# 4ment/physher

Hardware: AMD Instinct MI355X
Metric: lnL+gradient evals/sec, 1000-taxon GTR+G4 fp64, 1e6 site patterns (higher is better)
Workload: dtype f64

## Files before the change

include/physher_amd.h:

```cpp
#ifndef PHYSHER_AMD_H
#define PHYSHER_AMD_H

#include <stddef.h>
#include <stdint.h>

#ifdef __cplusplus
extern "C" {
#endif

typedef struct phyamd_engine phyamd_engine;

enum {
	PHYAMD_OK = 0,
	PHYAMD_EINVAL = -1,
	PHYAMD_EDEVICE = -2,
	PHYAMD_ENOMEM = -3,
	PHYAMD_EUNSUPPORTED = -4
};

enum { PHYAMD_RESCALE_NEVER = 0, PHYAMD_RESCALE_ALWAYS = 1, PHYAMD_RESCALE_AUTO = 2 };

enum {
	PHYAMD_GRAD_FOLD_ROOT_FREQS = 1,
	PHYAMD_GRAD_COMPAT_SCALED = 2
// ... 44 lines not shown
int phyamd_gradient(phyamd_engine *e, int flags, double *lnl, double *cat_gradient);
int phyamd_branch_gradient(phyamd_engine *e, int flags, const double *rates_without_mu , double *lnl,
                           double *branch_gradient);
int phyamd_log_likelihood_device(phyamd_engine *e, double *device_out);
int phyamd_gradient_device(phyamd_engine *e, int flags, double *device_out);
int phyamd_root_invariant_term(phyamd_engine *e, double *out);

#define PHYAMD_MAX_PARAMETERS 2048
int phyamd_set_rate_matrix_derivatives(phyamd_engine *e, int count, const double *dQ);
int phyamd_parameter_gradient(phyamd_engine *e, int flags, double *lnl, double *cat_gradient, double *parameter_gradient);
int phyamd_parameter_gradient_device(phyamd_engine *e, int flags, double *device_out);
int phyamd_root_frequency_term(phyamd_engine *e, double *out );
int phyamd_branch_log_likelihood(phyamd_engine *e, int node, double length, double *lnl, double *d1, double *d2);
int phyamd_branch_hessian_diagonal(phyamd_engine *e, int flags, double *lnl, double *d1, double *d2);
int phyamd_branch_hessian_diagonal_device(phyamd_engine *e, int flags, double *device_out);
int phyamd_gradient_batch(phyamd_engine *e, int flags, int32_t count, const double *branch_lengths, double *lnl, double *cat_gradient);
int phyamd_gradient_batch_trees(phyamd_engine *e, int flags, int32_t count, const int32_t *left, const int32_t *right,
                                const int32_t *roots, const double *branch_lengths, double *lnl, double *cat_gradient);
typedef struct { int32_t items_fast, items_sequential, chunks; int64_t scratch_bytes; double ms; } phyamd_batch_profile;
int phyamd_get_batch_profile(phyamd_engine *e, phyamd_batch_profile *out);
int phyamd_nni_log_likelihoods(phyamd_engine *e, int flags, const double *central_lengths ,
                               double *lnl , double *d1 , double *d2 );
typedef struct { int32_t candidates; int64_t scratch_bytes; double ms; } phyamd_nni_profile;
int phyamd_get_nni_profile(phyamd_engine *e, phyamd_nni_profile *out);
int phyamd_spr_log_likelihoods(phyamd_engine *e, int flags, int32_t count, const int32_t *prune ,
                               double *lnl );
typedef struct { int32_t prunes, chunks; int64_t candidates, scratch_bytes; double ms; } phyamd_spr_profile;
int phyamd_get_spr_profile(phyamd_engine *e, phyamd_spr_profile *out);
int phyamd_synchronize(phyamd_engine *e);

int phyamd_get_pattern_log_likelihoods(phyamd_engine *e, double *out );
int phyamd_get_partials(phyamd_engine *e, int node, int upper, double *out);
int phyamd_get_node_matrices(phyamd_engine *e, int node, int derivative, double *out );
int phyamd_is_rescaling(phyamd_engine *e);
int phyamd_set_rescaling(phyamd_engine *e, int policy);
int phyamd_set_keep_partials(phyamd_engine *e, int on);

typedef struct {
	double matrices_ms, lower_ms, upper_ms, reduce_ms;
	int32_t lower_launches, upper_launches;
	int64_t device_bytes;
	int32_t tiles;
} phyamd_profile;
int phyamd_set_reduction_levels(phyamd_engine *e, int levels);
int phyamd_set_profiling(phyamd_engine *e, int on);
int phyamd_get_profile(phyamd_engine *e, phyamd_profile *out);

#ifdef __cplusplus
}
#endif
#endif
```

physher_amd/_lib.py:

```python
from __future__ import annotations

import ctypes as C
import os

_HERE = os.path.dirname(os.path.abspath(__file__))
LIB_PATH = os.environ.get("PHYAMD_LIB") or os.path.join(_HERE, "libphysher_amd.so")

ABI_VERSION = 5

OK, EINVAL, EDEVICE, ENOMEM, EUNSUPPORTED = 0, -1, -2, -3, -4
RESCALE_NEVER, RESCALE_ALWAYS, RESCALE_AUTO = 0, 1, 2
GRAD_FOLD_ROOT_FREQS, GRAD_COMPAT_SCALED = 1, 2


class Config(C.Structure):
    _fields_ = [
        ("tip_count", C.c_int32), ("pattern_count", C.c_int32), ("state_count", C.c_int32),
        ("category_count", C.c_int32), ("device", C.c_int32), ("rescale", C.c_int32),
        ("max_device_bytes", C.c_int64), ("stream", C.c_void_p),
    ]


class Profile(C.Structure):
    _fields_ = [
# ... 31 lines not shown
    ("phyamd_set_branch_lengths", C.c_int, [_P, _P]),
    ("phyamd_set_branch_length", C.c_int, [_P, C.c_int, C.c_double]),
    ("phyamd_update_all_nodes", C.c_int, [_P]),
    ("phyamd_set_eigen", C.c_int, [_P, _P, _P, _P]),
    ("phyamd_set_frequencies", C.c_int, [_P, _P]),
    ("phyamd_set_category_rates", C.c_int, [_P, _P, _P]),
    ("phyamd_set_node_matrices", C.c_int, [_P, C.c_int, _P]),
    ("phyamd_set_matrices", C.c_int, [_P, _P]),
    ("phyamd_set_rate_matrix", C.c_int, [_P, _P]),
    ("phyamd_log_likelihood", C.c_int, [_P, C.POINTER(C.c_double)]),
    ("phyamd_gradient", C.c_int, [_P, C.c_int, C.POINTER(C.c_double), _P]),
    ("phyamd_branch_gradient", C.c_int, [_P, C.c_int, _P, C.POINTER(C.c_double), _P]),
    ("phyamd_gradient_device", C.c_int, [_P, C.c_int, _P]),
    ("phyamd_log_likelihood_device", C.c_int, [_P, _P]),
    ("phyamd_root_invariant_term", C.c_int, [_P, C.POINTER(C.c_double)]),
    ("phyamd_set_rate_matrix_derivatives", C.c_int, [_P, C.c_int, _P]),
    ("phyamd_parameter_gradient", C.c_int, [_P, C.c_int, C.POINTER(C.c_double), _P, _P]),
    ("phyamd_parameter_gradient_device", C.c_int, [_P, C.c_int, _P]),
    ("phyamd_root_frequency_term", C.c_int, [_P, _P]),
    ("phyamd_branch_log_likelihood", C.c_int, [_P, C.c_int, C.c_double, C.POINTER(C.c_double), C.POINTER(C.c_double), C.POINTER(C.c_double)]),
    ("phyamd_branch_hessian_diagonal", C.c_int, [_P, C.c_int, C.POINTER(C.c_double), _P, _P]),
    ("phyamd_branch_hessian_diagonal_device", C.c_int, [_P, C.c_int, _P]),
    ("phyamd_gradient_batch", C.c_int, [_P, C.c_int, C.c_int32, _P, _P, _P]),
    ("phyamd_gradient_batch_trees", C.c_int, [_P, C.c_int, C.c_int32, _P, _P, _P, _P, _P, _P]),
    ("phyamd_get_batch_profile", C.c_int, [_P, C.POINTER(BatchProfile)]),
    ("phyamd_nni_log_likelihoods", C.c_int, [_P, C.c_int, _P, _P, _P, _P]),
    ("phyamd_get_nni_profile", C.c_int, [_P, C.POINTER(NniProfile)]),
    ("phyamd_spr_log_likelihoods", C.c_int, [_P, C.c_int, C.c_int32, _P, _P]),
    ("phyamd_get_spr_profile", C.c_int, [_P, C.POINTER(SprProfile)]),
    ("phyamd_synchronize", C.c_int, [_P]),
    ("phyamd_get_pattern_log_likelihoods", C.c_int, [_P, _P]),
    ("phyamd_get_partials", C.c_int, [_P, C.c_int, C.c_int, _P]),
    ("phyamd_get_node_matrices", C.c_int, [_P, C.c_int, C.c_int, _P]),
    ("phyamd_is_rescaling", C.c_int, [_P]),
    ("phyamd_set_rescaling", C.c_int, [_P, C.c_int]),
    ("phyamd_set_keep_partials", C.c_int, [_P, C.c_int]),
    ("phyamd_set_reduction_levels", C.c_int, [_P, C.c_int]),
    ("phyamd_set_profiling", C.c_int, [_P, C.c_int]),
    ("phyamd_get_profile", C.c_int, [_P, C.POINTER(Profile)]),
    ("phyamd_store", C.c_int, [_P]),
    ("phyamd_restore", C.c_int, [_P]),
    ("phyamd_compress_patterns", C.c_int, [C.c_int, C.c_int32, C.c_int64, _P, _P, C.POINTER(C.c_int32), _P, _P]),
]

_lib = None


def load():
    global _lib
    if _lib is not None:
        return _lib
    if not os.path.exists(LIB_PATH):
        raise ImportError(f"{LIB_PATH} is missing: build the HIP engine first (make -C physher_amd/csrc); there is no CPU fallback")
    lib = C.CDLL(LIB_PATH)
    for name, res, args in SYMBOLS:
        fn = getattr(lib, name)
        fn.restype = res
        fn.argtypes = args
    if lib.phyamd_abi_version() != ABI_VERSION:
        raise ImportError(f"ABI mismatch: library {lib.phyamd_abi_version()} != binding {ABI_VERSION}")
    _lib = lib
    return lib


class EngineError(RuntimeError):
    def __init__(self, code, message):
# ... 3 lines not shown
```

physher_amd/csrc/phyamd_abi.inc:

```

#include <condition_variable>
#include <functional>
#include <mutex>
#include <thread>

namespace {

class ShardWorkers {
public:
	explicit ShardWorkers(int n) : done_(0), generation_(0), stop_(false) {
		for (int i = 0; i < n; i++) threads_.emplace_back([this, i] { loop(i); });
	}
	~ShardWorkers() {
		{
			std::lock_guard<std::mutex> lk(m_);
			stop_ = true;
			generation_++;
		}
		cv_.notify_all();
		for (auto &t : threads_) t.join();
	}
	void run(const std::function<void(int)> &fn) {
		std::unique_lock<std::mutex> lk(m_);
		fn_ = &fn;
// ... 561 lines not shown
}


int phyamd_get_pattern_log_likelihoods(phyamd_engine *g, double *out) {
	CHECK_GROUP(g);
	if (!out) return fail(PHYAMD_EINVAL, "null out");
	return for_shards(g, [&](Shard *s, int i) { return shard_get_pattern_log_likelihoods(s, out + g->offset[i]); });
}

int phyamd_get_partials(phyamd_engine *g, int node, int upper, double *out) {
	CHECK_GROUP(g);
	if (group_size(g) == 1) return shard_get_partials(g->shards[0], node, upper, out);
	if (!out) return fail(PHYAMD_EINVAL, "null out");
	int rc;
	std::vector<std::vector<double>> part(group_size(g));
	if ((rc = for_shards(g, [&](Shard *s, int i) {
		     part[i].resize((size_t)g->C * s->P * g->S);
		     return shard_get_partials(s, node, upper, part[i].data());
	     })))
		return rc;
	for (int i = 0; i < group_size(g); i++) {
		const size_t ps = (size_t)(g->offset[i + 1] - g->offset[i]);
		for (int c = 0; c < g->C; c++)
			std::memcpy(out + ((size_t)c * g->P + g->offset[i]) * g->S, part[i].data() + (size_t)c * ps * g->S, sizeof(double) * ps * g->S);
	}
	return PHYAMD_OK;
}

int phyamd_get_node_matrices(phyamd_engine *g, int node, int derivative, double *out) {
	CHECK_GROUP(g);
	return shard_get_node_matrices(g->shards[0], node, derivative, out);
}

int phyamd_is_rescaling(phyamd_engine *g) {
	CHECK_GROUP(g);
	int any = 0;
	for (Shard *s : g->shards) any |= shard_is_rescaling(s);
	return any;
}

int phyamd_get_profile(phyamd_engine *g, phyamd_profile *out) {
	CHECK_GROUP(g);
	if (!out) return fail(PHYAMD_EINVAL, "null out");
	int rc;
	if ((rc = shard_get_profile(g->shards[0], out))) return rc;
	for (int i = 1; i < group_size(g); i++) {
		phyamd_profile p;
		if ((rc = shard_get_profile(g->shards[i], &p))) return rc;
		out->matrices_ms = std::max(out->matrices_ms, p.matrices_ms);
		out->lower_ms = std::max(out->lower_ms, p.lower_ms);
		out->upper_ms = std::max(out->upper_ms, p.upper_ms);
		out->reduce_ms = std::max(out->reduce_ms, p.reduce_ms);
		out->device_bytes += p.device_bytes;
		out->tiles = std::max(out->tiles, p.tiles);
	}
	return PHYAMD_OK;
}

}
```

physher_amd/csrc/phyamd_engine.hip:

```cpp

#include <hip/hip_runtime.h>
#include <hipcub/hipcub.hpp>

#include <algorithm>
#include <chrono>
#include <cmath>
#include <cstdarg>
#include <cstdio>
#include <cstdlib>
#include <cstring>
#include <string>
#include <vector>

#include "physher_amd.h"

#define PHYAMD_ABI_VERSION 5

namespace {

thread_local std::string g_last_error;

int fail(int code, const char *fmt, ...) {
	char buf[512];
	va_list ap;
	va_start(ap, fmt);
	vsnprintf(buf, sizeof buf, fmt, ap);
	va_end(ap);
	g_last_error = buf;
	return code;
}

#define HIP_TRY(expr)                                                                                       \
	do {                                                                                                    \
		hipError_t err__ = (expr);                                                                          \
		if (err__ != hipSuccess)                                                                            \
			return fail(err__ == hipErrorOutOfMemory ? PHYAMD_ENOMEM : PHYAMD_EDEVICE, "%s: %s (%s:%d)", #expr, \
			            hipGetErrorString(err__), __FILE__, __LINE__);                                      \
	} while (0)

constexpr int WAVE = 64;
constexpr int PPT_LOWER = 2, PPT_UPPER = 8;
constexpr int UPPER_MIN_WAVES = 6;
constexpr int MAX_WAVES = 16;
// ... 47 lines not shown
```

physher_amd/csrc/phyamd_schedule.inc:

```

int bind_device(Shard *e) {
	HIP_TRY(hipSetDevice(e->device));
	return PHYAMD_OK;
}

size_t node_partial_doubles(const Shard *e) { return (size_t)e->C * e->S * (e->generic ? e->Pp : e->P); }
size_t lower_slots(const Shard *e) { return e->d_lower.size() / node_partial_doubles(e); }
size_t upper_slots_held(const Shard *e) { return e->d_upper.size() / node_partial_doubles(e); }

constexpr int WALK_CHUNKS = 3;
void build_walk_chunks(Shard *e) {
	const std::vector<NodeOp> &src = e->walk_upper_ops;
	const int n = (int)src.size(), N = e->N;
	e->walk_chunk_ops = src;
	e->walk_chunk_off.assign({0, n});
	e->walk_chunk_slots = 0;
	if (n == 0) return;
	std::vector<int> opi(N, -1), size(n, 1);
	for (int i = 0; i < n; i++) opi[src[i].parent] = i;
	for (int i = n - 1; i >= 0; i--)
		for (int ch : {src[i].left, src[i].right})
			if (opi[ch] >= 0) size[i] += size[opi[ch]];
	const int target = std::max(16, (n + WALK_CHUNKS - 1) / WALK_CHUNKS);
	std::vector<char> top(n, 0), cut(n, 0);
// ... 92 lines not shown
		for (int i = j; i < j + size[j]; i++) e->walk_chunk_ops.push_back(ops[i]);
		e->walk_chunk_off.push_back((int)e->walk_chunk_ops.size());
	}
	e->walk_chunk_slots = slots;
	e->walk_upper_slots = std::max(e->walk_upper_slots, slots);
}

void build_lower_walk_chunks(Shard *e) {
	const std::vector<NodeOp> &src = e->walk_lower_ops;
	const int n = (int)src.size(), N = e->N;
	e->walk_lower_chunk_ops = src;
	e->walk_lower_chunk_off.assign({0, n});
	if (n == 0) return;
	std::vector<int> opi(N, -1), size(n, 1);
	for (int i = 0; i < n; i++) opi[src[i].parent] = i;
	for (int i = 0; i < n; i++)
		for (int ch : {src[i].left, src[i].right})
			if (opi[ch] >= 0) size[i] += size[opi[ch]];
	const int target = std::max(16, (n + WALK_CHUNKS - 1) / WALK_CHUNKS);
	if (n < 32) return;
	std::vector<char> cut(n, 0), in_cut(n, 0);
	std::vector<int> stack{n - 1};
	while (!stack.empty()) {
		const int i = stack.back();
		stack.pop_back();
		for (int ch : {src[i].left, src[i].right}) {
			const int j = opi[ch];
			if (j < 0) continue;
			if (size[j] > target) stack.push_back(j);
			else cut[j] = 1;
		}
	}
	std::vector<NodeOp> out;
	std::vector<int> off{0}, cuts;
	for (int j = 0; j < n; j++)
		if (cut[j]) cuts.push_back(j);
	std::stable_sort(cuts.begin(), cuts.end(), [&](int a, int b) { return size[a] > size[b]; });
	for (int j : cuts) {
		for (int i = j - size[j] + 1; i <= j; i++) {
			in_cut[i] = 1;
			out.push_back(src[i]);
		}
		out[off.back()].carry_in = 0;
		off.push_back((int)out.size());
	}
	int prev = -1;
	for (int i = 0; i < n; i++) {
		if (in_cut[i]) continue;
		NodeOp op = src[i];
		const int jl = opi[op.left], jr = opi[op.right];
		const bool next_to_cut = (jl >= 0 && cut[jl]) || (jr >= 0 && cut[jr]);
		op.carry_in = prev >= 0 && prev == op.left ? 1 : prev >= 0 && prev == op.right ? 2 : 0;
		if (next_to_cut) op.lds_park &= ~3;
		out.push_back(op);
		prev = op.parent;
	}
	off.push_back((int)out.size());
	e->walk_lower_chunk_ops = out;
	e->walk_lower_chunk_off = off;
}

struct MaskPacker {
	std::vector<int> &rows;
	int row = -1, used = 32, entries = 8;
	explicit MaskPacker(std::vector<int> &r) : rows(r), row((int)r.size() / 8 - 1) {}
	void add(const int *tips, int &out_row, int &out_shift) {
		int span = 0, n = 0;
		for (int j = 0; j < 6; j++)
			if (tips[j] >= 0) {
				span = j + 1;
				n++;
			}
		const int bits = 1 + 4 * span;
		if (used + bits > 32 || entries + n > 8) {
			rows.insert(rows.end(), 8, -1);
			row++;
			used = 0;
			entries = 0;
		}
		out_row = row;
		out_shift = used;
		for (int j = 0; j < 6; j++)
			if (tips[j] >= 0) rows[(size_t)row * 8 + entries++] = tips[j] | (used + 1 + 4 * j) << 20 | used << 25;
		used += bits;
	}
};
// ... 206 lines not shown
		const int kinds[2] = {u.flags & 7, (u.flags >> 3) & 7};
		for (int side = 0; side < 2; side++)
			if (kinds[side] != CH_CORE) {
				int row, shift;
				packer.add(&e->stream_op_tips[(size_t)sop[o.parent] * 12 + 6 * side], row, shift);
				if (words[i] == 0) first_word[i] = row;
				last_word[i] = row;
				d.wsh |= shift << (5 * words[i]) | (row & 3) << (10 + 2 * words[i]);
				words[i]++;
			}
		int fl = (u.flags & 0x3F) | (u.flags & 0x00FF0000);
		d.lnode = moff(u.lnode);
		d.rnode = moff(u.rnode);
		d.self = o.parent == e->root ? 0 : moff(o.parent);
		d.store = (int64_t)o.core_parent * array_bytes;
		d.ls_store = (int64_t)o.core_parent * e->P * 8;
		for (int side = 0; side < 2; side++) {
			const int32_t *a = side ? u.ra : u.la;
			int32_t *m = side ? d.rm : d.lm;
			for (int j = 0; j < 5; j++) m[j] = 0;
			if (kinds[side] == CH_DEEP) {
				m[0] = moff(a[0]);
				m[1] = moff(a[4]);
				m[2] = moff(a[5]);
				m[3] = moff(a[9]);
			} else if (kinds[side] == CH_CHERRY_TIP)
				m[4] = moff(a[3]);
			if (kinds[side] != CH_CORE) continue;
			const int ch = side ? u.rnode : u.lnode;
			const bool is_left = ch == o.left;
			int src = 0;
			if (o.carry_in == (is_left ? 1 : 2)) src = 1;
			else if (o.lds_park & (is_left ? 1 : 2)) src = 2;
			else {
				(side ? d.mem_r : d.mem_l) = (int64_t)e->core_index[ch] * array_bytes;
				(side ? d.ls_r : d.ls_l) = (int64_t)e->core_index[ch] * e->P * 8;
			}
			fl |= src << (6 + 2 * side);
		}
		if (o.lds_park & 4) fl |= 1 << 10;
		pieces[i] = (kinds[0] != CH_CORE ? 1 : 0) | (kinds[1] != CH_CORE ? 2 : 0);
		d.flags = fl;
	}
	const int chunks = (int)e->walk_lower_chunk_off.size() - 1;
	for (int k = 0; k < chunks; k++) {
		const int b = e->walk_lower_chunk_off[k], en = e->walk_lower_chunk_off[k + 1];
		LowerChunk ch{0, 0, 0, 0, 0};
		int have = -1;
		auto fresh_rows = [&](int i, int &first) {
			if (words[i] == 0) return 0;
			first = have < 0 ? first_word[i] : std::max(first_word[i], have + 1);
			const int count = last_word[i] - first + 1;
			have = std::max(have, last_word[i]);
			return std::max(0, count);
		};
		if (b < en) {
			const int si = sop[e->walk_lower_chunk_ops[b].parent];
			int first = 0;
			const int count = fresh_rows(b, first);
			ch = LowerChunk{si, pieces[b], count, first & 3, (int64_t)first * row_bytes};
		}
		e->lstream_chunks.push_back(ch);
		for (int i = b; i < en; i++) {
			LowerDesc &d = e->lstream_desc[i];
			const bool last = i + 1 == en;
			const int sn = last ? 0 : sop[e->walk_lower_chunk_ops[i + 1].parent];
			d.nx_block = sn;
			int first = 0;
			const int count = last ? 0 : fresh_rows(i + 1, first);
			d.nx_words = (int64_t)first * row_bytes;
			d.flags |= count << 14;
			d.flags |= (first & 3) << 12;
			d.flags |= (last ? 0 : ((pieces[i + 1] & 2) ? 1 : 0)) << 24;
// ... 130 lines not shown
				int s;
				if (e->keep_partials) s = ch;
				else if (!free_slots.empty()) {
					s = free_slots.back();
					free_slots.pop_back();
				} else
					s = next_slot++;
				e->upper_slot[ch] = s;
				slots_of_depth[d + 1].push_back(s);
				(side ? op.upper_slot_right : op.upper_slot_left) = s;
			}
			e->upper_ops.push_back(op);
		}
		e->upper_level_off.push_back((int)e->upper_ops.size());
	}
	e->upper_slots = e->keep_partials ? N : next_slot;

	e->walking = e->walk_enabled && !e->generic && !e->keep_partials;
	e->gen_walking = e->walk_enabled && e->generic && e->S == 20 && !e->keep_partials && !e->scaling_on;
	e->walk_lower_ops.clear();
	e->walk_upper_ops.clear();
	e->walk_upper_slots = 0;
	if (e->walking || e->gen_walking) {
		std::vector<int> csize(N, 0), usize(N, 0);
		for (int i = N - 1; i >= 0; i--) {
			const int n = order[i];
			if (kind[n] == CH_CORE) csize[n] = 1 + csize[e->left[n]] + csize[e->right[n]];
			if (kind[n] == CH_CORE || kind[n] == CH_DEEP) usize[n] = 1 + usize[e->left[n]] + usize[e->right[n]];
		}
		struct Frame {
			int node, stage;
		};
		std::vector<uint8_t> two_core(N, 0);
		for (int i = N - 1; i >= 0; i--) {
			const int n = order[i];
			if (kind[n] != CH_CORE) continue;
			const int l = e->left[n], r = e->right[n];
			const bool lo = kind[l] == CH_CORE, ro = kind[r] == CH_CORE;
			two_core[n] = (lo && ro) || (lo && two_core[l]) || (ro && two_core[r]);
		}
		std::vector<int> lower_op_of(N, -1);
		std::vector<Frame> st{{e->root, 0}};
		while (!st.empty()) {
			Frame &f = st.back();
			const int n = f.node, l = e->left[n], r = e->right[n];
			const int first = csize[l] >= csize[r] ? l : r, second = first == l ? r : l;
			if (f.stage == 0) {
				f.stage = 1;
				if (kind[first] == CH_CORE) st.push_back({first, 0});
			} else if (f.stage == 1) {
				f.stage = 2;
				if (kind[second] == CH_CORE) st.push_back({second, 0});
			} else {
				NodeOp op = make_op(n);
				op.carry_in = 0;
				if (!e->walk_lower_ops.empty()) {
					const int prev = e->walk_lower_ops.back().parent;
					if (prev == l) op.carry_in = 1;
					else if (prev == r) op.carry_in = 2;
				}
				op.lds_park = 0;
				if (kind[first] == CH_CORE && kind[second] == CH_CORE && !two_core[second] && lower_op_of[first] >= 0) {
					e->walk_lower_ops[lower_op_of[first]].lds_park |= 4;
					op.lds_park |= first == l ? 1 : 2;
				}
				lower_op_of[n] = (int)e->walk_lower_ops.size();
				e->walk_lower_ops.push_back(op);
				st.pop_back();
			}
		}
		std::vector<uint8_t> parks(N, 0), in_lds(N, 0), in_lds2(N, 0);
		std::vector<int> height(N, 0);
		for (int i = N - 1; i >= 0; i--) {
			const int n = order[i];
			if (kind[n] != CH_CORE && kind[n] != CH_DEEP) continue;
			const int l = e->left[n], r = e->right[n];
			const bool lo = kind[l] == CH_CORE || kind[l] == CH_DEEP, ro = kind[r] == CH_CORE || kind[r] == CH_DEEP;
			parks[n] = (lo && ro) || (lo && parks[l]) || (ro && parks[r]);
			if (lo && ro) {
				const int first = usize[l] <= usize[r] ? l : r, second = first == l ? r : l;
				height[n] = std::max(1 + height[first], height[second]);
			} else
				height[n] = lo ? height[l] : ro ? height[r] : 0;
		}
		std::vector<int> free_w;
		int next_w = 0;
		std::vector<int> slot_of(N, -1);
		std::vector<int> stack2{e->root};
		int carried_node = -1;
		while (!stack2.empty()) {
			const int n = stack2.back();
			stack2.pop_back();
			NodeOp op = make_op(n);
			op.carry_in = (n != e->root && carried_node == n) ? 1 : 0;
			op.upper_slot_parent = -1;
			op.lds_park = 0;
			if (n != e->root && !op.carry_in) {
// ... 138 lines not shown
```

physher_amd/csrc/phyamd_shard.inc:

```

enum class LowerForm { Reference, Carried, CarriedExp2 };

struct ScheduleCounts { int core_count, upper_slots, widest; };

struct Shard {
	phyamd_config cfg{};
	DeviceBudget mem;
	DeviceBudget tile_mem{&mem};
	int T = 0, N = 0, P = 0, S = 0, C = 0, root = -1;
	int G = 1;
	bool generic = false;
	int Pp = 0;
	int nblk_root = 0;
	int nblk_lower = 0;
	int nblk_walk = 0, nblk_walk_upper = 0;
	int lower_walk_slots[2] = {0, 0};
	int gen_slots[3][2] = {};
	int lnl_blocks = 0;
	int grad_blocks = 0;
	size_t gpart_row = 0;
	struct State {
		bool all_dirty = true;
		std::vector<int> changed;
		bool force_root = false;
// ... 68 lines not shown
	bool stream_ambiguous = false;
	bool stream_unsupported = false;
	int stream_words = 0, stream_R = 0;
	DeviceArray<StreamDesc> d_stream_ops{&mem};
	DeviceArray<StreamChunk> d_stream_chunks{&mem};
	DeviceArray<int> d_stream_row_entries{&mem}, d_stream_site_tab{&mem}, d_stream_qnode{&mem}, d_oct_lo{&mem};
	DeviceArray<uint32_t> d_mstream{&tile_mem};
	size_t mstride = 0;
	unsigned long mstream_epoch = 0;
	std::vector<int> mstream_layout;
	double *d_gslab = nullptr;
	DeviceArray<double> d_oct{&mem};
	bool slab_walk_order = false;
	int reduce_levels = 3, seg_nb[2] = {-1, -1}, seg_levels[2] = {-1, -1};
	bool lnl_per_block = false;
	DeviceArray<double> d_Lc{&tile_mem};
	DeviceArray<double> d_imgs{&mem};
	DeviceArray<double> d_qp_mats{&mem};
	DeviceArray<double> d_qp_imgs{&mem};
	DeviceArray<double> d_inv_part{&tile_mem};
	int device = 0;
	hipStream_t stream = nullptr;
	bool own_stream = false;

	std::vector<int32_t> left, right, parent;
	std::vector<double> lengths, model, freqs, rates, props;
	std::vector<uint8_t> explicit_host;
	bool have_topology = false, have_lengths = false, have_eigen = false, have_freqs = false, have_rates = false, have_weights = false;
	std::vector<uint8_t> tip_set;
	bool scaling_on = false;
	LowerForm lower_form = LowerForm::Reference;
	bool reference_form_only = false;
	bool exp2_on = true, tform_on = true;
	DeviceArray<int> d_lexp{&tile_mem}, d_uexp{&tile_mem}, d_Ec{&tile_mem}, d_Eroot{&tile_mem};
	bool keep_partials = false;
	bool profiling = false;
	bool prof_pending = false, prof_with_upper = false;

	std::vector<NodeOp> lower_ops, upper_ops;
	std::vector<int> lower_level_off, upper_level_off;
	std::vector<int32_t> upper_slot;
	int upper_slots = 0;
	std::vector<int32_t> core_index;
	int core_count = 0;
	ScheduleCounts scaled_counts{0, 0, 1};
	bool have_scaled_counts = false;
	bool fusion_enabled = true, fused = false;
	std::vector<DeepDesc> deep_host;
	int deep_count = 0;

	DeviceArray<uint8_t> d_tipmask{&tile_mem};
	DeviceArray<unsigned long long> d_tipsets{&mem};
	std::vector<unsigned long long> tipsets_host;
	size_t tipsets_uploaded = 0;
	DeviceArray<double> d_lower{&tile_mem}, d_upper{&tile_mem}, d_mats{&mem}, d_dmats{&mem};
	DeviceArray<double> d_Q{&mem};
	DeviceArray<double> d_Qpi{&mem};
	std::vector<double> Q_host;
	bool have_Q = false;
	DeviceArray<double> d_tiptab{&mem};
	int np = 0;
	std::vector<double> dQ_host;
	DeviceArray<double> d_B{&mem};
	DeviceArray<double> d_dpm{&mem};
	DeviceArray<double> d_dptab{&mem};
	DeviceArray<double> d_ppart{&mem};
// ... 205 lines not shown
```

physher_amd/csrc/phyamd_shard_api.inc:

```

ScheduleCounts schedule_counts(const Shard *e) {
	ScheduleCounts c{e->core_count, std::max(e->upper_slots, e->walk_upper_slots), 1};
	for (size_t i = 0; i + 1 < e->lower_level_off.size(); i++) c.widest = std::max(c.widest, e->lower_level_off[i + 1] - e->lower_level_off[i]);
	for (size_t i = 0; i + 1 < e->upper_level_off.size(); i++) c.widest = std::max(c.widest, e->upper_level_off[i + 1] - e->upper_level_off[i]);
	return c;
}

double tile_working_set(const Shard *e, double p, bool exact, const ScheduleCounts &k) {
	const double pp = e->S == 4 ? p : std::ceil(p / 16.0) * 16.0, npd = (double)e->C * e->S * pp;
	const double per_pattern = (double)e->T * p + 8.0 * p * (3.0 + (e->S == 4 ? 0.0 : (double)e->C));
	const bool may_scale = e->cfg.rescale != PHYAMD_RESCALE_NEVER, exponents = may_scale && e->S == 4 && e->exp2_on;
	if (!exact) return 8.0 * (exponents ? 1.125 : 1.0) * ((e->S == 4 ? 0.5 : 1.6) * (double)(e->N - e->T) * npd + 2.0 * npd) + per_pattern;
	double doubles = (double)(std::max(1, k.core_count) + std::max(1, k.upper_slots)) * npd;
	if (may_scale) doubles += (double)std::max(1, k.core_count) * p + (e->S == 4 ? 0.0 : 5.0 * k.widest * e->C * p);
	if (exponents) doubles += 0.5 * ((double)(std::max(1, k.core_count) + std::max(1, k.upper_slots) + 1) * e->C * p + p);
	if (e->S == 4) doubles += (double)e->C * p;
	doubles += (double)e->N * e->C * (p / (WAVE * std::max(1, 4 / e->C)) + 1.0);
	if (e->S == 4) doubles += 2.0 * e->N * (p / (WAVE * PPT_UPPER) + 19.0) + 0.5 * p / 64.0;
	return 8.0 * doubles + per_pattern;
}

double tile_working_set(const Shard *e, double p, bool exact) {
	const double now = tile_working_set(e, p, exact, schedule_counts(e));
	return e->have_scaled_counts ? std::max(now, tile_working_set(e, p, exact, e->scaled_counts)) : now;
// ... 105 lines not shown
	e->N = 2 * e->T - 1;
	e->P = e->Ptot = cfg->pattern_count;
	e->S = cfg->state_count;
	e->C = cfg->category_count;
	if (cfg->device >= 0) e->device = cfg->device;
	else if (hipGetDevice(&e->device) != hipSuccess) e->device = 0;
	if (e->device >= ndev) {
		delete e;
		return fail(PHYAMD_EINVAL, "device %d out of range (%d visible)", cfg->device, ndev);
	}
	auto bail = [&](int rc) {
		shard_destroy(e);
		return rc;
	};
	int rc;
	{
		hipError_t err = hipSetDevice(e->device);
		if (err != hipSuccess) return bail(fail(PHYAMD_EDEVICE, "hipSetDevice(%d): %s", e->device, hipGetErrorString(err)));
	}
	if ((rc = choose_tiles(e, false))) return bail(rc);
	if (cfg->stream) e->stream = (hipStream_t)cfg->stream;
	else {
		hipError_t err = hipStreamCreateWithFlags(&e->stream, hipStreamNonBlocking);
		if (err != hipSuccess) return bail(fail(PHYAMD_EDEVICE, "hipStreamCreate: %s", hipGetErrorString(err)));
		e->own_stream = true;
	}
	e->scaling_on = cfg->rescale == PHYAMD_RESCALE_ALWAYS;
	if (const char *env = std::getenv("PHYAMD_FUSE")) e->fusion_enabled = std::atoi(env) != 0;
	if (const char *env = std::getenv("PHYAMD_WALK")) e->walk_enabled = std::atoi(env) != 0;
	if (const char *env = std::getenv("PHYAMD_GEN_FUSION")) e->generic_fusion = std::atoi(env) != 0;
	if (const char *env = std::getenv("PHYAMD_XCD_MAP")) e->xcd_map = std::atoi(env) != 0;
	if (const char *env = std::getenv("PHYAMD_SCALE_EXP2")) e->exp2_on = std::atoi(env) != 0;
	if (const char *env = std::getenv("PHYAMD_STREAM_TFORM")) e->tform_on = std::atoi(env) != 0;
	e->generic = e->S != 4;
	e->tip_set.assign(e->T, 0);
	e->tip_empty.assign(e->T, 0);
	e->mem.spare = &e->batch_mem;
	e->batch_max_patterns = BATCH_MAX_PATTERNS;
	if (const char *env = std::getenv("PHYAMD_BATCH_MAX_PATTERNS")) e->batch_max_patterns = std::atoi(env);
	if (const char *env = std::getenv("PHYAMD_BATCH_TRACE")) e->batch_trace = std::atoi(env) != 0;
	e->explicit_host.assign(e->N, 0);
	const size_t msz = (size_t)e->N * e->C * e->S * e->S;
	if (e->generic && ((rc = e->d_tipsets.ensure(256)) || (rc = e->d_imgs.ensure(((size_t)e->N * e->C + 2) * gen_image_doubles(e))))) return bail(rc);
	if (e->S == 20 && GenFuse<2>::QP) {
		if ((rc = e->d_qp_mats.ensure((size_t)e->T * e->C * e->S * e->S)) || (rc = e->d_qp_imgs.ensure((size_t)e->T * e->C * gen_image_doubles(e)))) return bail(rc);
	}
	if ((rc = e->d_mats.ensure(msz)) || (rc = e->d_dmats.ensure(msz)) || (rc = e->d_model.ensure((size_t)e->S + 2 * e->S * e->S)) ||
	    (rc = e->d_Q.ensure((size_t)e->S * e->S)))
		return bail(rc);
	if (!e->generic && (rc = e->d_tiptab.ensure((size_t)e->T * e->C * 64 + (size_t)e->N * 6))) return bail(rc);
	if ((rc = e->d_freqs.ensure(e->S)) || (rc = e->d_rates.ensure(e->C)) || (rc = e->d_props.ensure(e->C)) || (rc = e->d_lengths.ensure(e->N)) ||
	    (rc = e->d_result.ensure((size_t)1 + e->N * e->C + 2 * PHYAMD_MAX_PARAMETERS)) || (rc = e->d_explicit.ensure(e->N)) ||
	    (rc = e->d_row_valid.ensure((size_t)e->N * e->C)))
		return bail(rc);
	{
		hipError_t err = hipHostMalloc(reinterpret_cast<void **>(&e->h_result), sizeof(double) * ((size_t)2 + e->N * e->C + 2 * PHYAMD_MAX_PARAMETERS), hipHostMallocDefault);
		if (err != hipSuccess) return bail(fail(PHYAMD_EDEVICE, "hipHostMalloc: %s", hipGetErrorString(err)));
		err = hipMemsetAsync(e->d_explicit, 0, e->N, e->stream);
		if (err == hipSuccess) err = hipStreamSynchronize(e->stream);
		if (err != hipSuccess) return bail(fail(PHYAMD_EDEVICE, "memset: %s", hipGetErrorString(err)));
		for (auto &ev : e->ev) {
			err = hipEventCreate(&ev);
			if (err != hipSuccess) return bail(fail(PHYAMD_EDEVICE, "hipEventCreate: %s", hipGetErrorString(err)));
		}
	}
	if ((rc = allocate_pattern_storage(e))) return bail(rc);
// ... 1501 lines not shown
```

physher_amd/csrc/phyamd_walk4s.inc:

```

enum { HK_TIP = 0, HK_CHERRY = 1, HK_CHERRY_TIP = 2 };
enum { SU_CARRY = 0, SU_LDS = 1, SU_U = 2, SU_ROOT = 3 };

struct StreamOp {
	int32_t flags;
	int32_t parent;
	int32_t slot_parent, slot_left, slot_right;
	int32_t nx_mask_word;
	int32_t nx_a, nx_b;
	int32_t lnode, la[10];
	int32_t rnode, ra[10];
	int32_t nx_u;
	int32_t wsh;
};
static_assert(sizeof(StreamOp) == 128, "one StreamOp = 32 dwords");

struct StreamDesc {
	int32_t flags;
	int32_t parent, lnode, rnode;
	int32_t lm[5], rm[5];
	int64_t nx_words;
	int64_t nx_a, nx_b, nx_u;
	int64_t st_left, st_right;
	int32_t wsh;
// ... 465 lines not shown
			prev_tot = fold_sites<true>(ss.acc0, ss.acc1, ss.acc2);
		} else {
			if (kl == CH_CHERRY) s_descend<0, false, KEEP_BN>(x, ss, CH_CHERRY, op.lnode, op.lm[4], ul_terms, wL, bnl);
			if (kr == CH_CHERRY) s_descend<1, false, KEEP_BN>(x, ss, CH_CHERRY, op.rnode, op.rm[4], ur_terms, wR, bnr);
			prev_tot = fold_sites<false>(ss.acc0, ss.acc1, 0.0);
		}
		prev_off = soff;
		w0 = nw0;
		w1 = nw1;
		e_ul = e_l;
	}
	if (prev_off >= 0) *reinterpret_cast<double *>(slab + (unsigned)prev_off) = prev_tot;
}

struct LowerDesc {
	int32_t flags;
	int32_t nx_block;
	int32_t lnode, rnode, lm[5], rm[5];
	int64_t nx_words;
	int64_t store;
	int64_t mem_l, mem_r;
	int32_t wsh;
	int32_t self;
	int64_t ls_store, ls_l, ls_r;
	int32_t pad[2];
};
static_assert(sizeof(LowerDesc) == 128 && offsetof(LowerDesc, nx_words) == 56, "one LowerDesc = 32 dwords");
struct LowerChunk {
	int32_t block, pieces, mask_rows, slot;
	int64_t words;
};

constexpr int LSTREAM_MIN_WAVES = 5;
constexpr int LSTREAM_LDS_PER_WAVE = 2 * OPBLK_BYTES + 5 * WAVE * 4 + WAVE * 32;

__device__ __forceinline__ void dma_dword(const char *gsrc, lds_cptr dst) {
	__builtin_amdgcn_global_load_lds((const __attribute__((address_space(1))) void *)gsrc, (__attribute__((address_space(3))) void *)dst, 4, 0, 0);
}

template <bool AMBIG, int SCALE, bool TF = false>
__global__ __launch_bounds__(STREAM_WAVES *WAVE, SCALE == 1 ? 4 : LSTREAM_MIN_WAVES) void k_lower4_stream(
    const LowerDesc *__restrict__ ops, const LowerChunk *__restrict__ chunks, const int *__restrict__ chunk_off, int chunk_base, int nblocks, int P, int C, int nb,
    const uint32_t *__restrict__ mstream, size_t mstride, double *__restrict__ lower, const double *__restrict__ mats, const char *__restrict__ optab,
    const double *__restrict__ freqs, const double *__restrict__ props, double *__restrict__ Lc, int with_root, double *__restrict__ lscale, int xcd_map,
    int *__restrict__ Ec) {
	extern __shared__ double sh[];
	constexpr bool XCH = SCALE == 1, EXP2 = SCALE == 2;
	const int lane = threadIdx.x, wv = __builtin_amdgcn_readfirstlane(threadIdx.y);
	const unsigned vx = XCH ? blockIdx.x : xcd_position(blockIdx.x, gridDim.x, xcd_map);
	const int c = XCH ? wv : vx % C, blk = XCH ? (int)blockIdx.x : (int)(vx / C) * STREAM_WAVES + wv;
	if (blk >= nb) return;
	const size_t plane = (size_t)P * 4;
	const int k0 = blk * WAVE + lane;
	const bool valid = k0 < P;
	const unsigned k = valid ? k0 : P - 1;
	const unsigned poff = k * 32u, moff = (unsigned)k0 * 4u;
	const lds_cptr blocks = (lds_cptr)sh + (size_t)wv * LSTREAM_LDS_PER_WAVE;
	const lds_cptr wrows = blocks + 2 * OPBLK_BYTES;
	SX x{reinterpret_cast<const char *>(mats + (size_t)c * 16), blocks};
	const int chunk = chunk_base + blockIdx.y;
	const int op_begin = chunk_off[chunk], op_end = chunk_off[chunk + 1];
	const char *const optab_c = optab + (size_t)c * nblocks * OPBLK_BYTES + lane * 16;
	char *const lower_c = reinterpret_cast<char *>(lower + (size_t)c * plane);
	const char *const mstream_b = reinterpret_cast<const char *>(mstream) + moff;
	const size_t mrow = mstride * 4;
	const char *const hot = optab + (size_t)c * nblocks * OPBLK_BYTES + lane * 4;
	auto request_words = [&](int64_t off, int count, int slot) {
		dma_dword(count > 0 ? mstream_b + off : hot, wrows + (count > 0 ? slot : 4) * (WAVE * 4));
		dma_dword(count > 1 ? mstream_b + off + mrow : hot, wrows + (count > 1 ? ((slot + 1) & 3) : 4) * (WAVE * 4));
	};
	auto request_block = [&](int parity, int block, int pieces) {
		const char *src = optab_c + (size_t)block * OPBLK_BYTES;
		const lds_cptr dst = blocks + parity * OPBLK_BYTES;
		if (pieces & 1) dma_piece(src, dst);
		else dma_dword(hot, wrows + 4 * (WAVE * 4));
		if (pieces & 2) dma_piece(src + 1024, dst + 1024);
		else dma_dword(hot, wrows + 4 * (WAVE * 4));
	};
	if (op_begin < op_end) {
		const LowerChunk ch = chunks[chunk];
		request_block(op_begin & 1, ch.block, ch.pieces);
		request_words(ch.words, ch.mask_rows, ch.slot);
	}
	const lds_cptr stage = wrows + 5 * WAVE * 4;
	const bool valid_lo = blk * WAVE + (lane >> 1) < P, valid_hi = blk * WAVE + 32 + (lane >> 1) < P, full_block = (blk + 1) * WAVE <= P;
	auto store_result = [&](int64_t off, const d4 &v) {
		__attribute__((address_space(3))) dv2 *w = (__attribute__((address_space(3))) dv2 *)(stage + lane * 32);
		w[0] = dv2{v.x, v.y};
		w[1] = dv2{v.z, v.w};
		const dv2 lo = *(const __attribute__((address_space(3))) dv2 *)(stage + lane * 16), hi = *(const __attribute__((address_space(3))) dv2 *)(stage + 1024 + lane * 16);
		char *dst = lower_c + off + (size_t)blk * (WAVE * 32) + lane * 16;
		if (valid_lo) __builtin_nontemporal_store(lo, reinterpret_cast<dv2 *>(dst));
		if (valid_hi) __builtin_nontemporal_store(hi, reinterpret_cast<dv2 *>(dst + 1024));
	};
	d4 carry = d4{1., 1., 1., 1.}, parked = carry;
	double sfc = 0.0, sfp = 0.0;
	int efc = 0, efp = 0;
	double *const xbase = sh + (size_t)blockDim.y * (LSTREAM_LDS_PER_WAVE / 8);
	char *const lscale_k = XCH ? reinterpret_cast<char *>(lscale) + (size_t)k * 8 : nullptr;
	char *const lexp_k = EXP2 ? reinterpret_cast<char *>(lscale) + ((size_t)c * P + k) * 4 : nullptr;
	auto exp_at = [&](int64_t ls_off) -> int * { return reinterpret_cast<int *>(lexp_k + (ls_off >> 1) * C); };
	int64_t prev_store = 0, prev_ls = 0;
	bool have_prev = false, stored = false;
#pragma unroll 1
	for (int i = op_begin; i < op_end; i++) {
		LowerDesc op;
		{
			typedef const __attribute__((address_space(4))) int32_t *ciptr;
			const ciptr raw = (ciptr)(ops + i);
			int32_t *dst = reinterpret_cast<int32_t *>(&op);
#pragma unroll
			for (int j = 0; j < (SCALE ? 30 : TF ? 24 : 23); j++) dst[j] = raw[j];
		}
		if (!stored) asm volatile("s_waitcnt vmcnt(0)" ::: "memory");
		else if (EXP2 || (XCH && c == 0)) asm volatile("s_waitcnt vmcnt(3)" ::: "memory");
		else asm volatile("s_waitcnt vmcnt(2)" ::: "memory");
		const int fl = op.flags;
		const int kl = fl & 7, kr = (fl >> 3) & 7, sl = (fl >> 6) & 3, sr = (fl >> 8) & 3, nxw = (fl >> 14) & 3;
		x.tb = blocks + (i & 1) * OPBLK_BYTES;
		const unsigned w0 = *(const __attribute__((address_space(3))) unsigned *)(wrows + ((op.wsh >> 10) & 3) * (WAVE * 4) + lane * 4) >> (op.wsh & 31);
		const unsigned w1 = *(const __attribute__((address_space(3))) unsigned *)(wrows + ((op.wsh >> 12) & 3) * (WAVE * 4) + lane * 4) >> ((op.wsh >> 5) & 31);
		if (AMBIG) x.amb = __any((int)(((kl != CH_CORE || kr != CH_CORE ? w0 : 0u) | (kl != CH_CORE && kr != CH_CORE ? w1 : 0u)) & 1u)) != 0;
		if (i + 1 < op_end) {
			request_block((i + 1) & 1, op.nx_block, ((fl >> 25) & 1) | ((fl >> 23) & 2));
			request_words(op.nx_words, nxw, (fl >> 12) & 3);
		}
		stored = have_prev && full_block;
		if (have_prev) store_result(prev_store, carry);
		if (XCH && have_prev && c == 0 && valid) *reinterpret_cast<double *>(lscale_k + prev_ls) = sfc;
		if (EXP2 && have_prev && valid) __builtin_nontemporal_store(efc, exp_at(prev_ls));
		const unsigned wL = w0, wR = (kl != CH_CORE) ? w1 : w0;
		d4 bl, br, bn;
		any_value(bn);
		double sf_in = 0.0;
		int ef_in = 0;
		if (kl == CH_CORE) {
			d4 src = sl == 1 ? carry : parked;
			if (sl == 0) {
				src = load4(reinterpret_cast<const double *>(lower_c + op.mem_l + poff));
				if (XCH) sf_in += *reinterpret_cast<const double *>(lscale_k + op.ls_l);
				if (EXP2) ef_in += *exp_at(op.ls_l);
				stored = false;
			} else if (XCH) sf_in += sl == 1 ? sfc : sfp;
			else if (EXP2) ef_in += sl == 1 ? efc : efp;
			bl = TF ? src : matvec4_opt<false>(x.M(op.lnode), src);
		} else if (kl == CH_TIP) bl = x.site_tip<0, 0>(wL);
		else if (kl == CH_DEEP)
			bl = matvec4_opt<false>(x.M(op.lnode), mul4(s_half<0, 0>(x, (fl >> 16) & 3, op.lm[0], op.lm[1], wL), s_half<0, 3>(x, (fl >> 18) & 3, op.lm[2], op.lm[3], wL)));
		else bl = s_fringe_message<0, false>(x, kl, op.lnode, op.lm[4], wL, bn);
		if (kr == CH_CORE) {
			d4 src = sr == 1 ? carry : parked;
			if (sr == 0) {
				src = load4(reinterpret_cast<const double *>(lower_c + op.mem_r + poff));
				if (XCH) sf_in += *reinterpret_cast<const double *>(lscale_k + op.ls_r);
				if (EXP2) ef_in += *exp_at(op.ls_r);
				stored = false;
			} else if (XCH) sf_in += sr == 1 ? sfc : sfp;
			else if (EXP2) ef_in += sr == 1 ? efc : efp;
			br = TF ? src : matvec4_opt<false>(x.M(op.rnode), src);
		} else if (kr == CH_TIP) br = x.site_tip<1, 0>(wR);
		else if (kr == CH_DEEP)
			br = matvec4_opt<false>(x.M(op.rnode), mul4(s_half<1, 0>(x, (fl >> 20) & 3, op.rm[0], op.rm[1], wR), s_half<1, 3>(x, (fl >> 22) & 3, op.rm[2], op.rm[3], wR)));
		else br = s_fringe_message<1, false>(x, kr, op.rnode, op.rm[4], wR, bn);
		carry = mul4(bl, br);
		if (EXP2) efc = ef_in + exp2_rescale(carry);
		if (XCH) {
			double *xb = xbase + (size_t)(i & 1) * blockDim.y * WAVE;
			xb[c * WAVE + lane] = max4(carry);
			lds_barrier();
			double m = 0.0;
			for (int cc = 0; cc < C; cc++) m = fmax(m, xb[cc * WAVE + lane]);
			sfc = sf_in;
			if (m < SCALING_THRESHOLD) {
				carry = d4{carry.x / m, carry.y / m, carry.z / m, carry.w / m};
				sfc += log(m);
			}
		}
		if (TF && op.self) carry = matvec4_opt<false>(x.M(op.self), carry);
		if (fl & (1 << 10)) {
			parked = carry;
			sfp = sfc;
			efp = efc;
		}
		have_prev = !(fl & (1 << 11));
		prev_store = op.store;
		prev_ls = op.ls_store;
	}
	if (have_prev) store_result(prev_store, carry);
	if (XCH && have_prev && c == 0 && valid) *reinterpret_cast<double *>(lscale_k + prev_ls) = sfc;
	if (EXP2 && have_prev && valid) *exp_at(prev_ls) = efc;
	if (with_root && valid) {
		Lc[(size_t)c * P + k] = props[c] * (freqs[0] * carry.x + freqs[1] * carry.y + freqs[2] * carry.z + freqs[3] * carry.w);
		if (EXP2) Ec[(size_t)c * P + k] = efc;
	}
}

__global__ __launch_bounds__(64) void k_root_finish64(int P, int C, const double *__restrict__ Lc, const double *__restrict__ weights, double *__restrict__ pattern_lk,
                                                     double *__restrict__ w_over_L, double *__restrict__ lnl_part, const double *__restrict__ lscale_root,
                                                     const int *__restrict__ Ec, int *__restrict__ Eroot) {
	const int k = blockIdx.x * 64 + threadIdx.x;
	double term = 0.0;
	if (k < P) {
		double L = 0.0, ls = lscale_root ? lscale_root[k] : 0.0;
		if (Ec) {
			int E = Ec[k];
			for (int c = 1; c < C; c++) E = max(E, Ec[(size_t)c * P + k]);
			for (int c = 0; c < C; c++) L += ldexp(Lc[(size_t)c * P + k], Ec[(size_t)c * P + k] - E);
			Eroot[k] = E;
			ls = (double)E * 0.69314718055994530942;
		} else
			for (int c = 0; c < C; c++) L += Lc[(size_t)c * P + k];
		const double lk = log(L) + ls, w = weights[k];
		pattern_lk[k] = lk;
		w_over_L[k] = w / L;
		term = lk * w;
// ... 31 lines not shown
```

Baseline: 36.34.

## Add second register park slot to lower streaming walk to avoid partial reloads

Adds a second parked-carry register slot in the lower post-order streaming kernel, so a core child that would otherwise be re-read from global memory can stay in registers when the sibling subtree has exactly one nested two-core level. The schedule builder computes per-node park depth and sets new flag bits, and cut-chunk boundaries clear both park bits. This trades extra registers and branch selects for fewer partial-plane reloads. It also adds a diagnostic API and script that count the removed reloads, and an environment toggle that is on by default.

New measurement: 37.00, median of 6. +1.8%, better.

```diff
diff --git a/include/physher_amd.h b/include/physher_amd.h
--- a/include/physher_amd.h
+++ b/include/physher_amd.h
@@ -100,6 +100,8 @@
 int phyamd_get_pattern_log_likelihoods(phyamd_engine *e, double *out );
 int phyamd_get_partials(phyamd_engine *e, int node, int upper, double *out);
 int phyamd_get_node_matrices(phyamd_engine *e, int node, int derivative, double *out );
+int phyamd_post_order_parks(int32_t tip_count, const int32_t *left , const int32_t *right, int32_t root, int32_t second_slot,
+                            int32_t *out , int32_t capacity);
 int phyamd_is_rescaling(phyamd_engine *e);
 int phyamd_set_rescaling(phyamd_engine *e, int policy);
 int phyamd_set_keep_partials(phyamd_engine *e, int on);
diff --git a/physher_amd/_lib.py b/physher_amd/_lib.py
--- a/physher_amd/_lib.py
+++ b/physher_amd/_lib.py
@@ -87,6 +87,7 @@
     ("phyamd_get_pattern_log_likelihoods", C.c_int, [_P, _P]),
     ("phyamd_get_partials", C.c_int, [_P, C.c_int, C.c_int, _P]),
     ("phyamd_get_node_matrices", C.c_int, [_P, C.c_int, C.c_int, _P]),
+    ("phyamd_post_order_parks", C.c_int, [C.c_int32, _P, _P, C.c_int32, C.c_int32, _P, C.c_int32]),
     ("phyamd_is_rescaling", C.c_int, [_P]),
     ("phyamd_set_rescaling", C.c_int, [_P, C.c_int]),
     ("phyamd_set_keep_partials", C.c_int, [_P, C.c_int]),
diff --git a/physher_amd/csrc/phyamd_abi.inc b/physher_amd/csrc/phyamd_abi.inc
--- a/physher_amd/csrc/phyamd_abi.inc
+++ b/physher_amd/csrc/phyamd_abi.inc
@@ -617,6 +617,42 @@
 	return shard_get_node_matrices(g->shards[0], node, derivative, out);
 }
 
+int phyamd_post_order_parks(int32_t tip_count, const int32_t *left, const int32_t *right, int32_t root, int32_t second_slot, int32_t *out, int32_t capacity) {
+	if (tip_count < 2) return fail(PHYAMD_EINVAL, "tip_count must be >= 2 (got %d)", tip_count);
+	if (!left || !right) return fail(PHYAMD_EINVAL, "null left or right");
+	if (capacity < 0 || (capacity > 0 && !out)) return fail(PHYAMD_EINVAL, "null out with capacity %d", capacity);
+	std::unique_ptr<Shard> e(new Shard());
+	e->T = tip_count;
+	e->N = 2 * e->T - 1;
+	e->S = 4;
+	e->C = 1;
+	e->P = e->Ptot = 1;
+	e->root = root;
+	e->left.assign(left, left + e->N);
+	e->right.assign(right, right + e->N);
+	e->lower_park2_on = second_slot != 0;
+	int rc;
+	if ((rc = build_schedule(e.get()))) return rc;
+	const std::vector<NodeOp> &ops = e->walk_lower_chunk_ops;
+	const std::vector<int> &off = e->walk_lower_chunk_off;
+	std::vector<char> is_cut_root(e->N, 0);
+	for (size_t k = 1; k + 1 < off.size(); k++)
+		if (off[k] > off[k - 1]) is_cut_root[ops[off[k] - 1].parent] = 1;
+	int chunk = 0;
+	for (int i = 0; i < (int)ops.size() && i < capacity; i++) {
+		const NodeOp &o = ops[i];
+		while (i >= off[chunk + 1]) chunk++;
+		auto source = [&](int side) {
+			if ((side ? o.kind_right : o.kind_left) != CH_CORE) return -1;
+			return o.carry_in == side + 1 ? 1 : (o.lds_park & (1 << side)) ? 2 : (o.lds_park & (0x10 << side)) ? 3 : 0;
+		};
+		const int32_t rec[8] = {chunk, o.parent, o.left, o.right, source(0), source(1), ((o.lds_park & 4) ? 1 : 0) | ((o.lds_park & 0x40) ? 2 : 0),
+		                        (is_cut_root[o.left] ? 1 : 0) | (is_cut_root[o.right] ? 2 : 0)};
+		std::memcpy(out + (size_t)i * 8, rec, sizeof(rec));
+	}
+	return (int)ops.size();
+}
+
 int phyamd_is_rescaling(phyamd_engine *g) {
 	CHECK_GROUP(g);
 	int any = 0;
diff --git a/physher_amd/csrc/phyamd_engine.hip b/physher_amd/csrc/phyamd_engine.hip
--- a/physher_amd/csrc/phyamd_engine.hip
+++ b/physher_amd/csrc/phyamd_engine.hip
@@ -9,6 +9,7 @@
 #include <cstdio>
 #include <cstdlib>
 #include <cstring>
+#include <memory>
 #include <string>
 #include <vector>
 
diff --git a/physher_amd/csrc/phyamd_schedule.inc b/physher_amd/csrc/phyamd_schedule.inc
--- a/physher_amd/csrc/phyamd_schedule.inc
+++ b/physher_amd/csrc/phyamd_schedule.inc
@@ -148,13 +148,14 @@
 		}
 	}
 	std::vector<NodeOp> out;
-	std::vector<int> off{0}, cuts;
+	std::vector<int> off{0}, cuts, at(n, -1);
 	for (int j = 0; j < n; j++)
 		if (cut[j]) cuts.push_back(j);
 	std::stable_sort(cuts.begin(), cuts.end(), [&](int a, int b) { return size[a] > size[b]; });
 	for (int j : cuts) {
 		for (int i = j - size[j] + 1; i <= j; i++) {
 			in_cut[i] = 1;
+			at[i] = (int)out.size();
 			out.push_back(src[i]);
 		}
 		out[off.back()].carry_in = 0;
@@ -167,7 +168,15 @@
 		const int jl = opi[op.left], jr = opi[op.right];
 		const bool next_to_cut = (jl >= 0 && cut[jl]) || (jr >= 0 && cut[jr]);
 		op.carry_in = prev >= 0 && prev == op.left ? 1 : prev >= 0 && prev == op.right ? 2 : 0;
-		if (next_to_cut) op.lds_park &= ~3;
+		if (next_to_cut) {
+			for (int side = 0; side < 2; side++) {
+				const int j = side ? jr : jl;
+				if (op.lds_park & (side ? 2 : 1)) out[at[j]].lds_park &= ~4;
+				if (op.lds_park & (side ? 0x20 : 0x10)) out[at[j]].lds_park &= ~0x40;
+			}
+			op.lds_park &= ~0x33;
+		}
+		at[i] = (int)out.size();
 		out.push_back(op);
 		prev = op.parent;
 	}
@@ -440,13 +449,15 @@
 			int src = 0;
 			if (o.carry_in == (is_left ? 1 : 2)) src = 1;
 			else if (o.lds_park & (is_left ? 1 : 2)) src = 2;
-			else {
+			else if (o.lds_park & (is_left ? 0x10 : 0x20)) src = 3;
+			if (src == 0 || src == 3) {
 				(side ? d.mem_r : d.mem_l) = (int64_t)e->core_index[ch] * array_bytes;
 				(side ? d.ls_r : d.ls_l) = (int64_t)e->core_index[ch] * e->P * 8;
 			}
 			fl |= src << (6 + 2 * side);
 		}
 		if (o.lds_park & 4) fl |= 1 << 10;
+		if (o.lds_park & 0x40) fl |= 1 << 26;
 		pieces[i] = (kinds[0] != CH_CORE ? 1 : 0) | (kinds[1] != CH_CORE ? 2 : 0);
 		d.flags = fl;
 	}
@@ -643,12 +654,15 @@
 			int node, stage;
 		};
 		std::vector<uint8_t> two_core(N, 0);
+		std::vector<int> lparks(N, 0);
 		for (int i = N - 1; i >= 0; i--) {
 			const int n = order[i];
 			if (kind[n] != CH_CORE) continue;
 			const int l = e->left[n], r = e->right[n];
 			const bool lo = kind[l] == CH_CORE, ro = kind[r] == CH_CORE;
 			two_core[n] = (lo && ro) || (lo && two_core[l]) || (ro && two_core[r]);
+			if (lo && ro) lparks[n] = csize[l] >= csize[r] ? std::max(lparks[l], 1 + lparks[r]) : std::max(lparks[r], 1 + lparks[l]);
+			else lparks[n] = lo ? lparks[l] : ro ? lparks[r] : 0;
 		}
 		std::vector<int> lower_op_of(N, -1);
 		std::vector<Frame> st{{e->root, 0}};
@@ -671,9 +685,14 @@
 					else if (prev == r) op.carry_in = 2;
 				}
 				op.lds_park = 0;
-				if (kind[first] == CH_CORE && kind[second] == CH_CORE && !two_core[second] && lower_op_of[first] >= 0) {
-					e->walk_lower_ops[lower_op_of[first]].lds_park |= 4;
-					op.lds_park |= first == l ? 1 : 2;
+				if (kind[first] == CH_CORE && kind[second] == CH_CORE && lower_op_of[first] >= 0) {
+					if (!two_core[second]) {
+						e->walk_lower_ops[lower_op_of[first]].lds_park |= 4;
+						op.lds_park |= first == l ? 1 : 2;
+					} else if (e->lower_park2_on && lparks[second] == 1) {
+						e->walk_lower_ops[lower_op_of[first]].lds_park |= 0x40;
+						op.lds_park |= first == l ? 0x10 : 0x20;
+					}
 				}
 				lower_op_of[n] = (int)e->walk_lower_ops.size();
 				e->walk_lower_ops.push_back(op);
diff --git a/physher_amd/csrc/phyamd_shard.inc b/physher_amd/csrc/phyamd_shard.inc
--- a/physher_amd/csrc/phyamd_shard.inc
+++ b/physher_amd/csrc/phyamd_shard.inc
@@ -124,6 +124,7 @@
 	LowerForm lower_form = LowerForm::Reference;
 	bool reference_form_only = false;
 	bool exp2_on = true, tform_on = true;
+	bool lower_park2_on = true;
 	DeviceArray<int> d_lexp{&tile_mem}, d_uexp{&tile_mem}, d_Ec{&tile_mem}, d_Eroot{&tile_mem};
 	bool keep_partials = false;
 	bool profiling = false;
diff --git a/physher_amd/csrc/phyamd_shard_api.inc b/physher_amd/csrc/phyamd_shard_api.inc
--- a/physher_amd/csrc/phyamd_shard_api.inc
+++ b/physher_amd/csrc/phyamd_shard_api.inc
@@ -161,6 +161,7 @@
 	if (const char *env = std::getenv("PHYAMD_XCD_MAP")) e->xcd_map = std::atoi(env) != 0;
 	if (const char *env = std::getenv("PHYAMD_SCALE_EXP2")) e->exp2_on = std::atoi(env) != 0;
 	if (const char *env = std::getenv("PHYAMD_STREAM_TFORM")) e->tform_on = std::atoi(env) != 0;
+	if (const char *env = std::getenv("PHYAMD_LOWER_PARK2")) e->lower_park2_on = std::atoi(env) != 0;
 	e->generic = e->S != 4;
 	e->tip_set.assign(e->T, 0);
 	e->tip_empty.assign(e->T, 0);
diff --git a/physher_amd/csrc/phyamd_walk4s.inc b/physher_amd/csrc/phyamd_walk4s.inc
--- a/physher_amd/csrc/phyamd_walk4s.inc
+++ b/physher_amd/csrc/phyamd_walk4s.inc
@@ -521,6 +521,7 @@
 };
 
 constexpr int LSTREAM_MIN_WAVES = 5;
+constexpr int lstream_park_slots(bool ambig) { return ambig ? 1 : 2; }
 constexpr int LSTREAM_LDS_PER_WAVE = 2 * OPBLK_BYTES + 5 * WAVE * 4 + WAVE * 32;
 
 __device__ __forceinline__ void dma_dword(const char *gsrc, lds_cptr dst) {
@@ -534,7 +535,7 @@
     const double *__restrict__ freqs, const double *__restrict__ props, double *__restrict__ Lc, int with_root, double *__restrict__ lscale, int xcd_map,
     int *__restrict__ Ec) {
 	extern __shared__ double sh[];
-	constexpr bool XCH = SCALE == 1, EXP2 = SCALE == 2;
+	constexpr bool XCH = SCALE == 1, EXP2 = SCALE == 2, PARK2 = lstream_park_slots(AMBIG) > 1;
 	const int lane = threadIdx.x, wv = __builtin_amdgcn_readfirstlane(threadIdx.y);
 	const unsigned vx = XCH ? blockIdx.x : xcd_position(blockIdx.x, gridDim.x, xcd_map);
 	const int c = XCH ? wv : vx % C, blk = XCH ? (int)blockIdx.x : (int)(vx / C) * STREAM_WAVES + wv;
@@ -582,9 +583,9 @@
 		if (valid_lo) __builtin_nontemporal_store(lo, reinterpret_cast<dv2 *>(dst));
 		if (valid_hi) __builtin_nontemporal_store(hi, reinterpret_cast<dv2 *>(dst + 1024));
 	};
-	d4 carry = d4{1., 1., 1., 1.}, parked = carry;
-	double sfc = 0.0, sfp = 0.0;
-	int efc = 0, efp = 0;
+	d4 carry = d4{1., 1., 1., 1.}, parked = carry, parked2 = carry;
+	double sfc = 0.0, sfp = 0.0, sfp2 = 0.0;
+	int efc = 0, efp = 0, efp2 = 0;
 	double *const xbase = sh + (size_t)blockDim.y * (LSTREAM_LDS_PER_WAVE / 8);
 	char *const lscale_k = XCH ? reinterpret_cast<char *>(lscale) + (size_t)k * 8 : nullptr;
 	char *const lexp_k = EXP2 ? reinterpret_cast<char *>(lscale) + ((size_t)c * P + k) * 4 : nullptr;
@@ -605,7 +606,8 @@
 		else if (EXP2 || (XCH && c == 0)) asm volatile("s_waitcnt vmcnt(3)" ::: "memory");
 		else asm volatile("s_waitcnt vmcnt(2)" ::: "memory");
 		const int fl = op.flags;
-		const int kl = fl & 7, kr = (fl >> 3) & 7, sl = (fl >> 6) & 3, sr = (fl >> 8) & 3, nxw = (fl >> 14) & 3;
+		const int kl = fl & 7, kr = (fl >> 3) & 7, nxw = (fl >> 14) & 3;
+		const int sl = !PARK2 && ((fl >> 6) & 3) == 3 ? 0 : (fl >> 6) & 3, sr = !PARK2 && ((fl >> 8) & 3) == 3 ? 0 : (fl >> 8) & 3;
 		x.tb = blocks + (i & 1) * OPBLK_BYTES;
 		const unsigned w0 = *(const __attribute__((address_space(3))) unsigned *)(wrows + ((op.wsh >> 10) & 3) * (WAVE * 4) + lane * 4) >> (op.wsh & 31);
 		const unsigned w1 = *(const __attribute__((address_space(3))) unsigned *)(wrows + ((op.wsh >> 12) & 3) * (WAVE * 4) + lane * 4) >> ((op.wsh >> 5) & 31);
@@ -624,28 +626,28 @@
 		double sf_in = 0.0;
 		int ef_in = 0;
 		if (kl == CH_CORE) {
-			d4 src = sl == 1 ? carry : parked;
+			d4 src = sl == 1 ? carry : sl == 3 ? parked2 : parked;
 			if (sl == 0) {
 				src = load4(reinterpret_cast<const double *>(lower_c + op.mem_l + poff));
 				if (XCH) sf_in += *reinterpret_cast<const double *>(lscale_k + op.ls_l);
 				if (EXP2) ef_in += *exp_at(op.ls_l);
 				stored = false;
-			} else if (XCH) sf_in += sl == 1 ? sfc : sfp;
-			else if (EXP2) ef_in += sl == 1 ? efc : efp;
+			} else if (XCH) sf_in += sl == 1 ? sfc : sl == 3 ? sfp2 : sfp;
+			else if (EXP2) ef_in += sl == 1 ? efc : sl == 3 ? efp2 : efp;
 			bl = TF ? src : matvec4_opt<false>(x.M(op.lnode), src);
 		} else if (kl == CH_TIP) bl = x.site_tip<0, 0>(wL);
 		else if (kl == CH_DEEP)
 			bl = matvec4_opt<false>(x.M(op.lnode), mul4(s_half<0, 0>(x, (fl >> 16) & 3, op.lm[0], op.lm[1], wL), s_half<0, 3>(x, (fl >> 18) & 3, op.lm[2], op.lm[3], wL)));
 		else bl = s_fringe_message<0, false>(x, kl, op.lnode, op.lm[4], wL, bn);
 		if (kr == CH_CORE) {
-			d4 src = sr == 1 ? carry : parked;
+			d4 src = sr == 1 ? carry : sr == 3 ? parked2 : parked;
 			if (sr == 0) {
 				src = load4(reinterpret_cast<const double *>(lower_c + op.mem_r + poff));
 				if (XCH) sf_in += *reinterpret_cast<const double *>(lscale_k + op.ls_r);
 				if (EXP2) ef_in += *exp_at(op.ls_r);
 				stored = false;
-			} else if (XCH) sf_in += sr == 1 ? sfc : sfp;
-			else if (EXP2) ef_in += sr == 1 ? efc : efp;
+			} else if (XCH) sf_in += sr == 1 ? sfc : sr == 3 ? sfp2 : sfp;
+			else if (EXP2) ef_in += sr == 1 ? efc : sr == 3 ? efp2 : efp;
 			br = TF ? src : matvec4_opt<false>(x.M(op.rnode), src);
 		} else if (kr == CH_TIP) br = x.site_tip<1, 0>(wR);
 		else if (kr == CH_DEEP)
@@ -670,6 +672,11 @@
 			parked = carry;
 			sfp = sfc;
 			efp = efc;
+		}
+		if (PARK2 && (fl & (1 << 26))) {
+			parked2 = carry;
+			sfp2 = sfc;
+			efp2 = efc;
 		}
 		have_prev = !(fl & (1 << 11));
 		prev_store = op.store;
diff --git a/profiles/lower_park_count.py b/profiles/lower_park_count.py
--- /dev/null
+++ b/profiles/lower_park_count.py
@@ -0,0 +1,64 @@
+#!/usr/bin/env python3
+import json
+import os
+import sys
+
+import numpy as np
+
+sys.path.insert(0, os.path.dirname(os.path.dirname(os.path.abspath(__file__))))
+from physher_amd import _lib, synth
+
+PLANE_GB = 1e6 * 4 * 4 * 8 / 1e9
+MS_PER_GB = 0.37
+
+
+def parks(left, right, root, second_slot):
+    lib = _lib.load()
+    left = np.ascontiguousarray(left, dtype=np.int32)
+    right = np.ascontiguousarray(right, dtype=np.int32)
+    T = (len(left) + 1) // 2
+    out = np.zeros((T, 8), dtype=np.int32)
+    n = lib.phyamd_post_order_parks(T, left.ctypes.data, right.ctypes.data, int(root), int(second_slot), out.ctypes.data, T)
+    if n < 0:
+        raise RuntimeError(lib.phyamd_last_error().decode())
+    return out[:n]
+
+
+def count(left, right, root):
+    one, two = parks(left, right, root, 0), parks(left, right, root, 1)
+    assert (one[:, :4] == two[:, :4]).all()
+    res = {"ops": int(len(one)), "chunks": int(one[-1, 0]) + 1, "memory_one_slot": 0, "beside_cut": 0, "second_tier": 0, "deeper": 0,
+           "slot0": 0, "carried": 0}
+    for a, b in zip(one, two):
+        for side in (0, 1):
+            s1, s2 = int(a[4 + side]), int(b[4 + side])
+            res["slot0"] += s2 == 2
+            res["carried"] += s2 == 1
+            if s1 != 0:
+                continue
+            res["memory_one_slot"] += 1
+            if a[7] & (1 << side):
+                assert s2 == 0
+                res["beside_cut"] += 1
+            elif s2 == 3:
+                res["second_tier"] += 1
+            else:
+                assert s2 == 0
+                res["deeper"] += 1
+    res["memory_two_slots"] = res["beside_cut"] + res["deeper"]
+    res["removed_gb"] = round(res["second_tier"] * PLANE_GB, 3)
+    res["expected_gain_ms"] = round(res["second_tier"] * PLANE_GB * MS_PER_GB, 3)
+    return res
+
+
+def main():
+    taxa = int(sys.argv[1]) if len(sys.argv) > 1 else 1000
+    seed = int(sys.argv[2]) if len(sys.argv) > 2 else 1
+    tree = synth.random_tree(taxa, np.random.default_rng(seed))
+    res = {"taxa": taxa, "seed": seed}
+    res.update(count(tree.left, tree.right, tree.root))
+    print(json.dumps(res))
+
+
+if __name__ == "__main__":
+    main()
```
